# ramosian-glider/syzkaller

Hardware: AMD Instinct MI355X
Metric: coverage PCs triaged/sec vs corpus signal (+ % HBM roofline), 1/2/4/8 MI355X (higher is better)
Workload: dtype u32

## Files before the change

syzkaller_amd/csrc/sg_bucket.hip:

```cpp
#include "sg_part.h"

namespace sg {

#ifndef SG_BTHREADS
#define SG_BTHREADS 512
#endif
constexpr int kBThreads = SG_BTHREADS;
constexpr int kBWaves = kBThreads == 512 ? 6 : 8;
constexpr int kBU = 4;
constexpr uint32_t kHash = 8192;
constexpr uint32_t kMaxProbe = 31;
constexpr uint32_t kEmpty = 0xFFFFFFFFu;

struct BucketArgs {
  const uint32_t* in;
  const uint4* bdesc;
  const uint32_t* gbnd;
  uint32_t NG;
  uint32_t* mwords;
  const uint32_t* owords;
  uint32_t* nwords;
  uint8_t* rec_new;
  uint32_t* spill;
  uint32_t* nspill;
// ... 700 lines not shown
    cus = 256;
  const uint32_t grid = (uint32_t)(per_cu * cus);
  cache[key] = grid;
  return grid;
}

constexpr double kFsQueued = 0.9997;
static bool fs_split(sg_ctx* ctx) {
  const int64_t o = ctx->opt[kOptFlagSkip];
  if (o >= 0) return o != 0;
  m0f_poll(ctx);
  return ctx->m0f_queued >= kFsQueued;
}

int buckets_one(sg_ctx* ctx, const BucketPlan& bp, uint32_t* mwords, uint32_t* nwords, uint8_t* d_rec_new,
                const EmitArgs* emit, const uint32_t* owords) {
  const uint64_t nrec = bp.nrec;
  const uint32_t* gcount = bp.at<uint32_t>(ctx, kCB) + bp.ng;
  uint4* bdesc = bp.at<uint4>(ctx, kBD);
  uint32_t* nspill = bp.at<uint32_t>(ctx, kSP);
  const bool dbg = ctx->debug_part;
  BucketArgs ba{};
  ba.in = bp.at<uint32_t>(ctx, kV2);
  ba.bdesc = bdesc;
  ba.gbnd = bp.at<uint32_t>(ctx, kGB);
  ba.NG = (uint32_t)bp.NG;
  ba.mwords = mwords;
  ba.owords = owords;
  ba.nwords = nwords;
  ba.rec_new = d_rec_new;
  ba.nspill = nspill;
// ... 7 lines not shown
    ba.shard_cnt = emit->shard_cnt;
    ba.update = emit->update ? 1u : 0u;
    ba.gcur = emit->gcur;
    ba.goff = emit->goff;
  }
  uint32_t bgrid = persistent_grid(ctx, (const void*)k_bucket<false, 0>, kBThreads);
  const int64_t cap_blocks = ctx->opt[kOptBucketBlocks];
  if (cap_blocks > 0 && (uint64_t)cap_blocks < bgrid) bgrid = (uint32_t)cap_blocks;
  uint64_t* ddbg = nullptr;
  if (dbg) {
    SG_HIP(hipMalloc(&ddbg, (size_t)bgrid * 88));
    ba.dbg = ddbg;
  }
  const bool split = !emit && !dbg && d_rec_new && nrec <= kMaxLaunchRecords && fs_split(ctx);
  uint32_t* fsum = ba.ticket + 4;
  uint32_t* fcnt = (uint32_t*)ctx->dscal + 33;
  if (split) {
    if (!ctx->fs_ev) SG_HIP(hipEventCreateWithFlags(&ctx->fs_ev, hipEventDisableTiming));
    int rc = m0f_host_alloc(ctx);
    if (rc) return rc;
    SG_HIP(hipMemsetAsync(fcnt, 0, 4, ctx->stream));
  }
  SG_HIP(hipMemsetAsync(ba.ticket, 0, split ? 16 + kFsWords * 4 : 4, ctx->stream));
  SG_HIP(hipMemsetAsync(nspill, 0, 4, ctx->stream));
  ba.blist_b = bp.at<uint32_t>(ctx, kLB);
  ba.blist_q = bp.at<uint4>(ctx, kLQ);
  ba.nlist = bp.at<uint32_t>(ctx, kBP) + kNumBuckets;
  {
    ScopedTimer tm(ctx, "bucket_triage");
    if (split) {
      ba.win = 1;
      ba.win_shift = (uint32_t)ctx->opt[kOptFlagSkipSplit];
    }
    auto kb = emit  ? (emit->gcur ? k_bucket<false, 2> : k_bucket<false, 1>)
              : dbg ? k_bucket<true, 0>
                    : k_bucket<false, 0>;
    hipLaunchKernelGGL(kb, dim3(bgrid), dim3(kBThreads), 0, ctx->stream, ba);
    if (split) {
      hipLaunchKernelGGL(k_flag_summary, dim3(div_up(div_up(nrec, kFsRecs), 4)), dim3(256), 0, ctx->stream,
// ... 73 lines not shown
```

syzkaller_amd/csrc/sg_part.h:

```cpp
#pragma once

#include <algorithm>

#include "sg_internal.h"

namespace sg {

#ifndef SG_PT
#define SG_PT 16384
#endif
#ifndef SG_PTHREADS
#define SG_PTHREADS 1024
#endif
constexpr int kPT = SG_PT;
constexpr int kPThreads = SG_PTHREADS;
constexpr uint32_t kRecCap = 256;
constexpr uint32_t kGroupBits = 16;
constexpr uint32_t kGroupRecs = 1u << kGroupBits;
constexpr uint32_t kMaxGroups = 256;
static_assert(kGroupRecs % kRecCap == 0, "group boundaries must be tile cuts");
constexpr uint32_t kNumBuckets = 1u << 16;
constexpr uint32_t kBucketWords = 2048;
static_assert(kMaxLaunchRecords == (uint64_t)kMaxGroups * kGroupRecs, "records per partitioned launch");

// ... 19 lines not shown
}

constexpr uint32_t kFsBits = 12, kFsRecs = 1u << kFsBits;
constexpr uint32_t kFsWords = (uint32_t)(kMaxLaunchRecords >> kFsBits) / 32;
static_assert(kFsWords * 32ull * kFsRecs == kMaxLaunchRecords, "summary covers a launch's records");

constexpr uint64_t kSliceEntries = 1ull << 30;

struct RecSlice {
  uint64_t r0, r1, e0, e1;
};

enum Region : int {
  kTS, kTR, kGT,
  kH1, kO1, kV1, kB1,
  kNC, kCB,
  kCS, kCG, kCF,
  kCD, kDT,
  kBD, kGB,
  kH2, kO2, kV2,
  kSP, kTK,
  kBN, kBP,
  kLB, kLQ,
  kSC, kKM,
  kRegions
};
static_assert(kRegions <= sizeof(WsPlan::off) / sizeof(size_t), "the plan's regions fit WsPlan");

struct BucketPlan {
  uint64_t n, nrec, nA, nB, T, NG, ng, gmax;
  WsPlan p;
  size_t base = 0;
  BucketPlan(uint64_t n_, uint64_t nrec_);
  void rebase(size_t b) { base += b; }
  template <typename E>
  E* at(sg_ctx* ctx, Region r) const { return (E*)ws_at(ctx, base + p.off[r]); }
};

int partition_pass1(sg_ctx* ctx, const uint32_t* d_vals, const uint64_t* d_off, size_t ws_base, bool reserved,
                    BucketPlan& bp, bool trace, bool plane);
int partition_pass2(sg_ctx* ctx, const BucketPlan& bp, bool plane = true);
int partition_one(sg_ctx* ctx, const uint32_t* d_vals, const uint64_t* d_off, size_t ws_base, bool reserved,
                  BucketPlan& bp, bool trace = false);
int buckets_one(sg_ctx* ctx, const BucketPlan& bp, uint32_t* mwords, uint32_t* nwords, uint8_t* d_rec_new,
                const EmitArgs* emit, const uint32_t* owords = nullptr);
int m0_filter(sg_ctx* ctx, const BucketPlan& bp, uint32_t* mwords, uint32_t* nwords, uint8_t* d_rec_new, bool* done);
bool m0f_try(sg_ctx* ctx);
void m0f_poll(sg_ctx* ctx);
int m0f_note_partitioned(sg_ctx* ctx, const uint8_t* d_rec_new, uint64_t nrec);
int m0f_host_alloc(sg_ctx* ctx);
int record_slices(sg_ctx* ctx, const uint64_t* d_off, uint64_t nrec, std::vector<RecSlice>& out,
                  uint64_t lim = kSliceEntries);
int bucket_triage_one(sg_ctx* ctx, uint32_t* mwords, uint32_t* nwords, const uint32_t* d_vals, const uint64_t* d_off,
                      uint64_t n, uint64_t nrec, uint8_t* d_rec_new, const EmitArgs* emit = nullptr, size_t ws_base = 0,
                      bool trace = false);

}
```

syzkaller_amd/csrc/sg_part_triage.hip:

```cpp
#include "sg_part.h"

namespace sg {

int bucket_triage_one(sg_ctx* ctx, uint32_t* mwords, uint32_t* nwords, const uint32_t* d_vals, const uint64_t* d_off,
                      uint64_t n, uint64_t nrec, uint8_t* d_rec_new, const EmitArgs* emit, size_t ws_base, bool trace) {
  if (n == 0) return SG_OK;
  if (nrec == 0) {
    set_error("bucket triage: signal entries without records");
    return SG_EINVAL;
  }
  BucketPlan bp(n, nrec);
  if (emit || ws_base) {
    int rc = partition_one(ctx, d_vals, d_off, ws_base, ws_base != 0, bp, trace);
    if (rc) return rc;
    return buckets_one(ctx, bp, mwords, nwords, d_rec_new, emit);
  }
  const bool filter = m0f_try(ctx);
  int rc = partition_pass1(ctx, d_vals, d_off, 0, false, bp, trace, !filter);
  if (rc) return rc;
  if (filter) {
    bool done = false;
    rc = m0_filter(ctx, bp, mwords, nwords, d_rec_new, &done);
    if (rc || done) return rc;
  }
  rc = partition_pass2(ctx, bp, !filter);
  if (!rc) rc = buckets_one(ctx, bp, mwords, nwords, d_rec_new, nullptr);
  if (!rc) rc = m0f_note_partitioned(ctx, d_rec_new, nrec);
  return rc;
}

__global__ void k_rebase(const uint64_t* __restrict__ off, uint64_t n, uint64_t base, uint64_t* __restrict__ out) {
  const uint64_t i = (uint64_t)blockIdx.x * blockDim.x + threadIdx.x;
  if (i < n) out[i] = off[i] - base;
}

int rebase_offsets(sg_ctx* ctx, const uint64_t* d_off, uint64_t n, uint64_t base, uint64_t* d_out) {
  hipLaunchKernelGGL(k_rebase, dim3(div_up(n, 256)), dim3(256), 0, ctx->stream, d_off, n, base, d_out);
  SG_HIP(hipGetLastError());
  return SG_OK;
}

// ... 92 lines not shown

int record_slice_cuts(sg_ctx* ctx, const uint64_t* d_off, uint64_t nrec, uint64_t lim, std::vector<uint64_t>& cuts) {
  std::vector<RecSlice> sl;
  const int rc = record_slices(ctx, d_off, nrec, sl, lim);
  cuts.clear();
  for (const RecSlice& x : sl) cuts.insert(cuts.end(), {x.r0, x.r1, x.e0, x.e1});
  return rc;
}

int bucket_triage(sg_ctx* ctx, uint32_t* mwords, uint32_t* nwords, const uint32_t* d_vals, const uint64_t* d_off,
                  uint64_t n, uint64_t nrec, uint8_t* d_rec_new, bool trace) {
  if (nrec >= 0xFFFFFFFFull || n >= 0xFFFFFFFFull - 2 * kPT) {
    set_error("bucket triage: a batch holds < 2^32 signal entries and < 2^32 - 1 records");
    return SG_EINVAL;
  }
  if (nrec) SG_HIP(hipMemsetAsync(d_rec_new, 0, nrec, ctx->stream));
  const uint64_t m = ctx->max_launch_recs;
  if (nrec <= m && n <= kSliceEntries)
    return bucket_triage_one(ctx, mwords, nwords, d_vals, d_off, n, nrec, d_rec_new, nullptr, 0, trace);
  std::vector<RecSlice> sl;
  int rc = record_slices(ctx, d_off, nrec, sl);
  if (rc) return rc;
  const size_t need = nrec + sl.size();
  if (ctx->slice_off_cap < need) {
    SG_HIP(hipStreamSynchronize(ctx->stream));
    if (ctx->slice_off) SG_HIP(hipFree(ctx->slice_off));
    ctx->slice_off = nullptr;
    ctx->slice_off_cap = 0;
    SG_HIP(hipMalloc(&ctx->slice_off, need * 8));
    ctx->slice_off_cap = need;
  }
  size_t at = 0;
  for (const RecSlice& x : sl) {
    const uint64_t nr = x.r1 - x.r0;
// ... 38 lines not shown
```

syzkaller_amd/csrc/sg_partition.hip:

```cpp
#include "sg_part.h"

namespace sg {

constexpr int kPWaves = kPThreads / 64;
constexpr int kPerWave = kPT / kPWaves;
constexpr int kSteps = kPerWave / 64;

__device__ __forceinline__ uint32_t xcd_tile(uint32_t bid, uint32_t g) {
  const uint32_t x = bid & 7, q = g >> 3, r = g & 7;
  return (x < r ? x * (q + 1) : r * (q + 1) + (x - r) * q) + (bid >> 3);
}

struct Cuts {
  uint64_t nA, step, nB, n;
  const uint64_t* rec_off;
  uint64_t nrec;
  uint32_t* start;
  uint32_t* aux;
  __device__ __forceinline__ uint64_t B(uint64_t j) const { return rec_off[(j + 1) * kRecCap]; }
  __device__ __forceinline__ uint64_t countB(uint64_t x) const {
    uint64_t lo = 0, hi = nB;
    while (lo < hi) {
      const uint64_t mid = (lo + hi) >> 1;
      if (B(mid) < x)
        lo = mid + 1;
      else
        hi = mid;
    }
    return lo;
  }
};

__global__ void k_cuts(Cuts c) {
  const uint64_t i = (uint64_t)blockIdx.x * blockDim.x + threadIdx.x;
  const uint64_t total = c.nA + c.nB;
  if (i > total) return;
  if (i == total) {
    c.start[total] = (uint32_t)c.n;
    return;
  }
  uint64_t x, rank;
  if (i < c.nA) {
    x = i * c.step;
    rank = i + c.countB(x);
  } else {
    const uint64_t j = i - c.nA;
    x = c.B(j);
    const uint64_t a = x / c.step + 1;
    rank = j + (a < c.nA ? a : c.nA);
  }
  c.start[rank] = (uint32_t)x;
  const uint64_t xe = x < c.n ? x : (c.n ? c.n - 1 : 0);
  c.aux[rank] = (uint32_t)sgd::seg_search(c.rec_off, 0, c.nrec - 1, xe);
}

__global__ void k_group_tiles(const uint64_t* __restrict__ rec_off, uint64_t nA, uint32_t NG, uint32_t T,
                              uint32_t* __restrict__ gt) {
  const uint32_t g = blockIdx.x * blockDim.x + threadIdx.x;
  if (g > NG) return;
  if (g == 0 || g == NG) {
    gt[g] = g ? T : 0u;
    return;
  }
  const uint64_t a = rec_off[(uint64_t)g * kGroupRecs] / kPT + 1;
  gt[g] = (uint32_t)((uint64_t)g * (kGroupRecs / kRecCap) - 1 + (a < nA ? a : nA));
}

__device__ __forceinline__ uint32_t group_start(const uint32_t* goff1, uint32_t T, uint32_t NG, const uint32_t* gt,
                                                uint64_t j) {
  return goff1[(j / NG) * T + gt[j % NG]];
}

__global__ void k_group_chunks(const uint32_t* __restrict__ goff1, uint32_t T, uint32_t NG,
                               const uint32_t* __restrict__ gt, uint64_t ng, uint32_t* __restrict__ nch) {
  const uint64_t j = (uint64_t)blockIdx.x * blockDim.x + threadIdx.x;
  if (j >= ng) return;
  const uint32_t sz = group_start(goff1, T, NG, gt, j + 1) - group_start(goff1, T, NG, gt, j);
  nch[j] = (sz + kPT - 1) / kPT;
}

__global__ void k_chunk_list(const uint32_t* __restrict__ goff1, uint32_t T, uint32_t NG,
                             const uint32_t* __restrict__ gt, uint64_t ng,
                             const uint32_t* __restrict__ cbase, uint64_t gmax, uint32_t* __restrict__ cstart,
                             uint32_t* __restrict__ cgov, uint32_t* __restrict__ cfirst) {
  const uint64_t i = (uint64_t)blockIdx.x * blockDim.x + threadIdx.x;
  const uint32_t G = cbase[ng], n = goff1[256ull * T];
  if (i < ng) {
    const uint32_t g0 = group_start(goff1, T, NG, gt, i), g1 = group_start(goff1, T, NG, gt, i + 1);
    uint32_t c = cbase[i];
    for (uint32_t e = g0; e < g1; e += kPT, c++) {
      cstart[c] = e;
      cgov[c] = (uint32_t)i;
    }
  }
  if (i >= G && i <= gmax) {
    cstart[i] = n;
    cgov[i] = (uint32_t)(ng - 1);
  }
  if (i <= 256) cfirst[i] = i < 256 ? cbase[i * NG] : G;
}


__global__ void k_chunk_desc(const uint32_t* __restrict__ cstart, const uint32_t* __restrict__ cgov,
                             const uint32_t* __restrict__ gcount, uint64_t gmax, const uint32_t* __restrict__ goff1,
                             uint32_t T, uint32_t NG, const uint32_t* __restrict__ gt, uint4* __restrict__ desc,
                             uint2* __restrict__ dtile) {
  const uint64_t bid = (uint64_t)blockIdx.x * blockDim.x + threadIdx.x;
  if (bid >= gmax) return;
  const uint32_t G = *gcount;
  if (bid < G) {
    const uint32_t c = xcd_tile((uint32_t)bid, G), s0 = cstart[c], s1 = cstart[c + 1], j = cgov[c];
    const uint32_t* row = goff1 + (uint64_t)(j / NG) * T;
    const uint32_t lo = gt[j % NG], hi = gt[j % NG + 1];
    desc[bid] = make_uint4(s0, s1, j, c);
    dtile[bid] = make_uint2(last_le(row, lo, hi, s0), last_le(row, lo, hi, s1 - 1) + 1);
  } else {
    desc[bid] = make_uint4(0, 0, 0, 0);
    dtile[bid] = make_uint2(0, 0);
  }
}

constexpr int kHistQ = kPT / 4 / kPThreads;

__global__ __launch_bounds__(kPThreads) void k_p1_hist(const uint32_t* __restrict__ v,
                                                       const uint32_t* __restrict__ start, uint32_t* __restrict__ hist) {
  __shared__ uint32_t cnt[256];
// ... 519 lines not shown
__global__ __launch_bounds__(kPThreads) __attribute__((amdgpu_waves_per_eu(8, 8))) void k_p2_scatter(P2Args a) {
  __shared__ uint32_t stage[kPT];
  __shared__ uint32_t cnt[256];
  __shared__ uint32_t gbase[256];
  __shared__ SegLds<uint16_t> L;
  const uint4 dsc = a.desc[blockIdx.x];
  const uint2 dt = a.dtile[blockIdx.x];
  const uint32_t s0 = dsc.x, s1 = dsc.y;
  if (s0 >= s1) return;
  if (s1 - s0 == (uint32_t)kPT)
    p2_chunk<true>(a, stage, cnt, gbase, L, s0, s1, dsc.z, dsc.w, dt);
  else
    p2_chunk<false>(a, stage, cnt, gbase, L, s0, s1, dsc.z, dsc.w, dt);
}

__global__ void k_bucket_compact(const uint4* __restrict__ bdesc, const uint32_t* __restrict__ lpos,
                                 uint32_t* __restrict__ blist_b, uint4* __restrict__ blist_q) {
  const uint32_t b = blockIdx.x * blockDim.x + threadIdx.x;
  if (b >= kNumBuckets) return;
  const uint4 q = bdesc[b];
  if (q.x < q.y) {
    blist_b[lpos[b]] = b;
    blist_q[lpos[b]] = q;
  }
}

__global__ void k_bucket_desc(const uint32_t* __restrict__ goff2, const uint32_t* __restrict__ gcount,
                              const uint32_t* __restrict__ cfirst, uint4* __restrict__ bdesc, uint32_t* __restrict__ nz) {
  const uint32_t b = blockIdx.x * blockDim.x + threadIdx.x;
  if (b >= kNumBuckets) return;
  const uint32_t d = b >> 8, f = b & 255, c0 = cfirst[d], nch = cfirst[d + 1] - c0;
  const uint32_t* row = goff2 + (uint64_t)f * *gcount + c0;
  const uint32_t lo = row[0], hi = row[nch];
  bdesc[b] = make_uint4(lo, hi, c0, nch);
  nz[b] = lo < hi ? 1u : 0u;
}

__global__ void k_bucket_groups(const uint32_t* __restrict__ goff2, const uint32_t* __restrict__ gcount,
                                const uint32_t* __restrict__ cbase, uint32_t NG, uint32_t* __restrict__ gbnd) {
  const uint64_t i = (uint64_t)blockIdx.x * blockDim.x + threadIdx.x;
  if (i >= (uint64_t)kNumBuckets * NG) return;
  const uint32_t b = (uint32_t)(i / NG), g = (uint32_t)(i % NG);
  gbnd[i] = goff2[(uint64_t)(b & 255) * *gcount + cbase[(b >> 8) * NG + g]];
}

__global__ void k_top_plane(const uint32_t* __restrict__ v1, uint64_t n, uint8_t* __restrict__ b1) {
  for (uint64_t i = ((uint64_t)blockIdx.x * blockDim.x + threadIdx.x) * 4; i < n;
       i += (uint64_t)gridDim.x * blockDim.x * 4) {
    if (i + 4 <= n && ((uintptr_t)(v1 + i) & 15) == 0) {
      const uint4 q = *reinterpret_cast<const uint4*>(v1 + i);
      *reinterpret_cast<uint32_t*>(b1 + i) = (q.x >> 24) | ((q.y >> 24) << 8) | ((q.z >> 24) << 16) | (q.w & 0xFF000000u);
    } else {
      for (uint64_t k = i; k < i + 4 && k < n; k++) b1[k] = (uint8_t)(v1[k] >> 24);
    }
  }
}

constexpr int kScanThreads = 1024;
constexpr int kScanPer = 16;
constexpr uint32_t kScanTile = kScanThreads * kScanPer;

__device__ __forceinline__ uint32_t block_excl_scan(uint32_t v, uint32_t* wsum, uint32_t* total) {
  const int tid = threadIdx.x, lane = tid & 63, w = tid >> 6;
  uint32_t incl = v;
#pragma unroll
  for (int o = 1; o < 64; o <<= 1) {
    const uint32_t y = __shfl_up(incl, o);
    if (lane >= o) incl += y;
  }
  if (lane == 63) wsum[w] = incl;
  __syncthreads();
  if (tid < 64) {
    const uint32_t x = tid < (int)(blockDim.x >> 6) ? wsum[tid] : 0u;
    uint32_t wi = x;
#pragma unroll
    for (int o = 1; o < 64; o <<= 1) {
      const uint32_t y = __shfl_up(wi, o);
      if (lane >= o) wi += y;
    }
    if (tid < (int)(blockDim.x >> 6)) wsum[tid] = wi - x;
    if (tid == 63) *total = wi;
  }
  __syncthreads();
  return wsum[w] + incl - v;
}
// ... 14 lines not shown
    for (int k = 0; k < kScanPer; k++) {
      const uint64_t i = base + (uint64_t)k * kScanThreads + threadIdx.x;
      s += i < n ? in[i] : 0u;
    }
  }
  for (int o = 32; o; o >>= 1) s += __shfl_down(s, o);
  if ((threadIdx.x & 63) == 0) wsum[threadIdx.x >> 6] = s;
  __syncthreads();
  if (threadIdx.x == 0) {
    uint32_t t = 0;
    for (int w = 0; w < kScanThreads / 64; w++) t += wsum[w];
    sums[blockIdx.x] = t;
  }
}

__global__ __launch_bounds__(kScanThreads) void k_scan32_top(uint32_t* __restrict__ sums, uint64_t nb) {
  __shared__ uint32_t wsum[16];
  __shared__ uint32_t tot;
  uint32_t carry = 0;
  for (uint64_t b0 = 0; b0 < nb; b0 += kScanThreads) {
    const uint64_t i = b0 + threadIdx.x;
    const uint32_t v = i < nb ? sums[i] : 0u;
    const uint32_t ex = block_excl_scan(v, wsum, &tot);
    if (i < nb) sums[i] = carry + ex;
    carry += tot;
    __syncthreads();
  }
}

__global__ __launch_bounds__(kScanThreads) void k_scan32_apply(const uint32_t* __restrict__ in, uint64_t n,
                                                               const uint32_t* __restrict__ n_dev, uint32_t mul,
                                                               const uint32_t* __restrict__ sums,
                                                               uint32_t* __restrict__ out) {
  __shared__ uint32_t wsum[16];
  __shared__ uint32_t tot;
  n = scan_n(n, n_dev, mul);
  const uint64_t b_last = n ? (n - 1) / kScanTile : 0;
  if (blockIdx.x > b_last) return;
  const uint64_t base = (uint64_t)blockIdx.x * kScanTile + (uint64_t)threadIdx.x * kScanPer;
  const bool full = base + kScanPer <= n;
  uint32_t v[kScanPer];
  uint32_t s = 0;
  if (full) {
#pragma unroll
    for (int k = 0; k < kScanPer; k += 4) {
      const uint4 q = *reinterpret_cast<const uint4*>(in + base + k);
      v[k] = q.x;
      v[k + 1] = q.y;
      v[k + 2] = q.z;
      v[k + 3] = q.w;
    }
  } else {
#pragma unroll
    for (int k = 0; k < kScanPer; k++) v[k] = base + k < n ? in[base + k] : 0u;
  }
#pragma unroll
  for (int k = 0; k < kScanPer; k++) s += v[k];
  uint32_t run = (sums ? sums[blockIdx.x] : 0u) + block_excl_scan(s, wsum, &tot);
  uint32_t o[kScanPer];
#pragma unroll
  for (int k = 0; k < kScanPer; k++) {
    o[k] = run;
    run += v[k];
  }
  if (full) {
#pragma unroll
    for (int k = 0; k < kScanPer; k += 4)
      *reinterpret_cast<uint4*>(out + base + k) = make_uint4(o[k], o[k + 1], o[k + 2], o[k + 3]);
  } else {
#pragma unroll
    for (int k = 0; k < kScanPer; k++)
      if (base + k < n) out[base + k] = o[k];
  }
// ... 6 lines not shown
                  const uint32_t* n_dev = nullptr, uint32_t mul = 1) {
  ScopedTimer tm(ctx, "scan");
  const uint64_t nb = (n + kScanTile - 1) / kScanTile;
  if (nb == 0) {
    SG_HIP(hipMemsetAsync(out, 0, 4, ctx->stream));
    return SG_OK;
  }
  if (nb == 1) {
    hipLaunchKernelGGL(k_scan32_apply, dim3(1), dim3(kScanThreads), 0, ctx->stream, in, n, n_dev, mul,
                       (const uint32_t*)nullptr, out);
    SG_HIP(hipGetLastError());
    return SG_OK;
  }
  hipLaunchKernelGGL(k_scan32_reduce, dim3((uint32_t)nb), dim3(kScanThreads), 0, ctx->stream, in, n, n_dev, mul,
                     scratch);
  hipLaunchKernelGGL(k_scan32_top, dim3(1), dim3(kScanThreads), 0, ctx->stream, scratch, nb);
  hipLaunchKernelGGL(k_scan32_apply, dim3((uint32_t)nb), dim3(kScanThreads), 0, ctx->stream, in, n, n_dev, mul,
                     scratch, out);
  SG_HIP(hipGetLastError());
  return SG_OK;
}

BucketPlan::BucketPlan(uint64_t n_, uint64_t nrec_) : n(n_), nrec(nrec_) {
  nA = (n + kPT - 1) / kPT;
  nB = nrec ? (nrec - 1) / kRecCap : 0;
  T = nA + nB;
  NG = nrec ? (nrec - 1) / kGroupRecs + 1 : 1;
  ng = 256 * NG;
  gmax = ng + nA;
  const uint64_t nb = kNumBuckets;
  const size_t bytes[] = {
      (T + 1) * 4, (T + 1) * 4, (NG + 1) * 4,
      256 * T * 4, (256 * T + 1) * 4, n * 4, n + 64,
      ng * 4, (ng + 1) * 4,
      (gmax + 1) * 4, (gmax + 1) * 4, 257 * 4,
      gmax * 16, gmax * 8,
      nb * 16, nb * NG * 4,
      256 * gmax * 4, (256 * gmax + 1) * 4, n * 4 + 64,
      (nb + 1) * 4, 16 + kFsWords * 4,
      nb * 4, (nb + 1) * 4,
      nb * 4, nb * 16,
      scan32_ws(256 * (gmax > T ? gmax : T)), T * (kPT / 8),
  };
  static_assert(sizeof(bytes) / sizeof(bytes[0]) == kRegions, "one size per region");
  for (size_t b : bytes) p.add(b);
}

size_t bucket_plan_bytes(uint64_t n, uint64_t nrec) { return BucketPlan(n, nrec).p.total; }

int partition_pass1(sg_ctx* ctx, const uint32_t* d_vals, const uint64_t* d_off, size_t ws_base, bool reserved,
                    BucketPlan& bp, bool trace, bool plane) {
  if (256 * bp.gmax >= 0xFFFFFFFFull || bp.NG > kMaxGroups) {
    set_error("bucket triage: batch too large");
    return SG_EINVAL;
  }
  int rc = reserved ? SG_OK : ws_reserve(ctx, ws_base + bp.p.total);
  if (rc) return rc;
  if (ctx->ws_cap < ws_base + bp.p.total) {
    set_error("bucket triage: workspace not reserved");
    return SG_EINVAL;
  }
  bp.rebase(ws_base);
  uint32_t* tstart = bp.at<uint32_t>(ctx, kTS);
  uint32_t* trec = bp.at<uint32_t>(ctx, kTR);
  uint32_t* hist1 = bp.at<uint32_t>(ctx, kH1);
  uint32_t* goff1 = bp.at<uint32_t>(ctx, kO1);
  uint64_t* keep = bp.at<uint64_t>(ctx, kKM);
  const uint32_t T = (uint32_t)bp.T, NG = (uint32_t)bp.NG;
  const bool dbg = ctx->debug_part;
  const Cuts c1{bp.nA, kPT, bp.nB, bp.n, d_off, bp.nrec, tstart, trec};
  hipLaunchKernelGGL(k_cuts, dim3(div_up(bp.T + 1, 256)), dim3(256), 0, ctx->stream, c1);
  hipLaunchKernelGGL(k_group_tiles, dim3(div_up(bp.NG + 1, 256)), dim3(256), 0, ctx->stream, d_off, bp.nA, NG, T,
                     bp.at<uint32_t>(ctx, kGT));
  {
    ScopedTimer tm(ctx, "p1_hist");
    if (trace)
      hipLaunchKernelGGL(k_hist_trace, dim3(T), dim3(kPThreads), 0, ctx->stream, d_vals, d_off, bp.nrec,
                         (const uint32_t*)tstart, (const uint32_t*)trec, T, hist1, keep);
    else if (((uintptr_t)d_vals & 15) == 0)
      hipLaunchKernelGGL(k_hist_rep<false>, dim3(T), dim3(kPThreads), 0, ctx->stream, d_vals,
                         (const uint32_t*)tstart, (const uint4*)nullptr, T, (const uint32_t*)nullptr, hist1);
    else
      hipLaunchKernelGGL(k_p1_hist, dim3(T), dim3(kPThreads), 0, ctx->stream, d_vals,
                         (const uint32_t*)tstart, hist1);
  }
  rc = scan32(ctx, hist1, goff1, 256 * bp.T, bp.at<uint32_t>(ctx, kSC));
  if (rc) return rc;
  P1Args a1{d_vals, d_off, bp.nrec, tstart, trec, T, goff1, hist1, bp.at<uint32_t>(ctx, kV1),
// ... 9 lines not shown
    auto k1 = dbg ? (trace ? k_p1_scatter<true, true> : k_p1_scatter<true, false>)
                  : (trace ? k_p1_scatter<false, true> : k_p1_scatter<false, false>);
    hipLaunchKernelGGL(k1, dim3(T), dim3(kPThreads), 0, ctx->stream, a1);
  }
  if (dbg) {
    unsigned long long h[8];
    SG_HIP(hipMemcpy(h, p1dbg, 64, hipMemcpyDeviceToHost));
    SG_HIP(hipFree(p1dbg));
    fprintf(stderr, "sg p1_scatter per tile (cycles, wave 0): load+meta %.0f build+lookup %.0f rank %.0f stage %.0f "
            "write %.0f (tiles %llu)\n", (double)h[0] / h[5], (double)h[1] / h[5], (double)h[2] / h[5],
            (double)h[3] / h[5], (double)h[4] / h[5], h[5]);
  }
  return SG_OK;
}

int partition_pass2(sg_ctx* ctx, const BucketPlan& bp, bool plane) {
  const uint32_t* gt = bp.at<uint32_t>(ctx, kGT);
  const uint32_t* goff1 = bp.at<uint32_t>(ctx, kO1);
  uint32_t* v1 = bp.at<uint32_t>(ctx, kV1);
  uint8_t* b1 = bp.at<uint8_t>(ctx, kB1);
  uint32_t* nch = bp.at<uint32_t>(ctx, kNC);
  uint32_t* cbase = bp.at<uint32_t>(ctx, kCB);
  uint32_t* cstart = bp.at<uint32_t>(ctx, kCS);
  uint32_t* cgov = bp.at<uint32_t>(ctx, kCG);
  uint32_t* cfirst = bp.at<uint32_t>(ctx, kCF);
  uint4* cdesc = bp.at<uint4>(ctx, kCD);
  uint2* dtile = bp.at<uint2>(ctx, kDT);
  uint4* bdesc = bp.at<uint4>(ctx, kBD);
  uint32_t* hist2 = bp.at<uint32_t>(ctx, kH2);
  uint32_t* goff2 = bp.at<uint32_t>(ctx, kO2);
  uint32_t* scr = bp.at<uint32_t>(ctx, kSC);
  uint32_t* bnz = bp.at<uint32_t>(ctx, kBN);
  uint32_t* blpos = bp.at<uint32_t>(ctx, kBP);
  const uint32_t T = (uint32_t)bp.T, G = (uint32_t)bp.gmax, NG = (uint32_t)bp.NG;
  const uint32_t* gcount = cbase + bp.ng;
  if (!plane) {
    hipLaunchKernelGGL(k_top_plane, dim3((uint32_t)std::min<uint64_t>(4096, div_up(bp.n, 1024))), dim3(256), 0,
                       ctx->stream, (const uint32_t*)v1, bp.n, b1);
    SG_HIP(hipGetLastError());
  }
  hipLaunchKernelGGL(k_group_chunks, dim3(div_up(bp.ng, 256)), dim3(256), 0, ctx->stream, goff1, T, NG, gt, bp.ng,
                     nch);
  int rc = scan32(ctx, nch, cbase, bp.ng, scr);
  if (rc) return rc;
  hipLaunchKernelGGL(k_chunk_list, dim3(div_up((bp.ng > bp.gmax ? bp.ng : bp.gmax) + 1, 256)), dim3(256), 0,
                     ctx->stream, goff1, T, NG, gt, bp.ng, (const uint32_t*)cbase, bp.gmax, cstart, cgov, cfirst);
  hipLaunchKernelGGL(k_chunk_desc, dim3(div_up(bp.gmax, 256)), dim3(256), 0, ctx->stream, (const uint32_t*)cstart,
                     (const uint32_t*)cgov, gcount, bp.gmax, goff1, T, NG, gt, cdesc, dtile);
  {
    ScopedTimer tm(ctx, "p2_hist");
    hipLaunchKernelGGL(k_hist_bytes, dim3(G), dim3(kHBThreads), 0, ctx->stream, (const uint8_t*)b1,
                       (const uint4*)cdesc, gcount, hist2);
  }
  rc = scan32(ctx, hist2, goff2, 256 * bp.gmax, scr, gcount, 256);
  if (rc) return rc;
  P2Args a2{v1, cdesc, dtile, gcount, goff1, bp.at<uint32_t>(ctx, kTR), T, NG, goff2, hist2, bp.at<uint32_t>(ctx, kV2)};
  {
    ScopedTimer tm(ctx, "p2_scatter");
    hipLaunchKernelGGL(k_p2_scatter, dim3(G), dim3(kPThreads), 0, ctx->stream, a2);
  }
  hipLaunchKernelGGL(k_bucket_desc, dim3(kNumBuckets / 256), dim3(256), 0, ctx->stream, (const uint32_t*)goff2,
                     gcount, (const uint32_t*)cfirst, bdesc, bnz);
  hipLaunchKernelGGL(k_bucket_groups, dim3(div_up((uint64_t)kNumBuckets * NG, 256)), dim3(256), 0, ctx->stream,
                     (const uint32_t*)goff2, gcount, (const uint32_t*)cbase, NG, bp.at<uint32_t>(ctx, kGB));
  rc = scan32(ctx, bnz, blpos, kNumBuckets, scr);
  if (rc) return rc;
  hipLaunchKernelGGL(k_bucket_compact, dim3(kNumBuckets / 256), dim3(256), 0, ctx->stream, (const uint4*)bdesc,
                     (const uint32_t*)blpos, bp.at<uint32_t>(ctx, kLB), bp.at<uint4>(ctx, kLQ));
  SG_HIP(hipGetLastError());
  return SG_OK;
}

int partition_one(sg_ctx* ctx, const uint32_t* d_vals, const uint64_t* d_off, size_t ws_base, bool reserved,
                  BucketPlan& bp, bool trace) {
  const int rc = partition_pass1(ctx, d_vals, d_off, ws_base, reserved, bp, trace, true);
  return rc ? rc : partition_pass2(ctx, bp);
}

}
```

Baseline: 134.7 billion.

## Fuse partition bookkeeping kernels and fold memsets into kernels to cut launches

Merges the cut and group-tile kernels into one launch, which also zeroes the record-new flags in place of a separate memset. The chunk count, scan and list kernels become a single-block chunk kernel, with chunk descriptors found by binary search over the chunk bases. The bucket descriptor, group, scan and compact steps become two kernels that use per-block counts, and the ticket, spill and flag-count scalars are zeroed inside them, so the memsets in buckets_one are skipped. The top-level scan kernel is removed by having each apply block sum the preceding block totals itself. The goal is fewer small launches and memsets per batch, at the cost of a serial single-block chunk scan and redundant prefix summation in each block.

```diff
diff --git a/syzkaller_amd/csrc/sg_bucket.hip b/syzkaller_amd/csrc/sg_bucket.hip
--- a/syzkaller_amd/csrc/sg_bucket.hip
+++ b/syzkaller_amd/csrc/sg_bucket.hip
@@ -738,7 +738,7 @@
 }
 
 int buckets_one(sg_ctx* ctx, const BucketPlan& bp, uint32_t* mwords, uint32_t* nwords, uint8_t* d_rec_new,
-                const EmitArgs* emit, const uint32_t* owords) {
+                const EmitArgs* emit, const uint32_t* owords, bool scalars_zeroed) {
   const uint64_t nrec = bp.nrec;
   const uint32_t* gcount = bp.at<uint32_t>(ctx, kCB) + bp.ng;
   uint4* bdesc = bp.at<uint4>(ctx, kBD);
@@ -776,15 +776,17 @@
   }
   const bool split = !emit && !dbg && d_rec_new && nrec <= kMaxLaunchRecords && fs_split(ctx);
   uint32_t* fsum = ba.ticket + 4;
-  uint32_t* fcnt = (uint32_t*)ctx->dscal + 33;
+  uint32_t* fcnt = fs_count(ctx);
   if (split) {
     if (!ctx->fs_ev) SG_HIP(hipEventCreateWithFlags(&ctx->fs_ev, hipEventDisableTiming));
     int rc = m0f_host_alloc(ctx);
     if (rc) return rc;
-    SG_HIP(hipMemsetAsync(fcnt, 0, 4, ctx->stream));
-  }
-  SG_HIP(hipMemsetAsync(ba.ticket, 0, split ? 16 + kFsWords * 4 : 4, ctx->stream));
-  SG_HIP(hipMemsetAsync(nspill, 0, 4, ctx->stream));
+    if (!scalars_zeroed) SG_HIP(hipMemsetAsync(fcnt, 0, 4, ctx->stream));
+  }
+  if (!scalars_zeroed) {
+    SG_HIP(hipMemsetAsync(ba.ticket, 0, split ? 16 + kFsWords * 4 : 4, ctx->stream));
+    SG_HIP(hipMemsetAsync(nspill, 0, 4, ctx->stream));
+  }
   ba.blist_b = bp.at<uint32_t>(ctx, kLB);
   ba.blist_q = bp.at<uint4>(ctx, kLQ);
   ba.nlist = bp.at<uint32_t>(ctx, kBP) + kNumBuckets;
diff --git a/syzkaller_amd/csrc/sg_part.h b/syzkaller_amd/csrc/sg_part.h
--- a/syzkaller_amd/csrc/sg_part.h
+++ b/syzkaller_amd/csrc/sg_part.h
@@ -57,8 +57,8 @@
 enum Region : int {
   kTS, kTR, kGT,
   kH1, kO1, kV1, kB1,
-  kNC, kCB,
-  kCS, kCG, kCF,
+  kCB,
+  kCF,
   kCD, kDT,
   kBD, kGB,
   kH2, kO2, kV2,
@@ -81,12 +81,13 @@
 };
 
 int partition_pass1(sg_ctx* ctx, const uint32_t* d_vals, const uint64_t* d_off, size_t ws_base, bool reserved,
-                    BucketPlan& bp, bool trace, bool plane);
-int partition_pass2(sg_ctx* ctx, const BucketPlan& bp, bool plane = true);
+                    BucketPlan& bp, bool trace, bool plane, uint8_t* clear_flags = nullptr);
+int partition_pass2(sg_ctx* ctx, const BucketPlan& bp, bool plane = true, uint32_t* zero_fcnt = nullptr);
 int partition_one(sg_ctx* ctx, const uint32_t* d_vals, const uint64_t* d_off, size_t ws_base, bool reserved,
                   BucketPlan& bp, bool trace = false);
 int buckets_one(sg_ctx* ctx, const BucketPlan& bp, uint32_t* mwords, uint32_t* nwords, uint8_t* d_rec_new,
-                const EmitArgs* emit, const uint32_t* owords = nullptr);
+                const EmitArgs* emit, const uint32_t* owords = nullptr, bool scalars_zeroed = false);
+inline uint32_t* fs_count(sg_ctx* ctx) { return (uint32_t*)ctx->dscal + 33; }
 int m0_filter(sg_ctx* ctx, const BucketPlan& bp, uint32_t* mwords, uint32_t* nwords, uint8_t* d_rec_new, bool* done);
 bool m0f_try(sg_ctx* ctx);
 void m0f_poll(sg_ctx* ctx);
@@ -96,6 +97,6 @@
                   uint64_t lim = kSliceEntries);
 int bucket_triage_one(sg_ctx* ctx, uint32_t* mwords, uint32_t* nwords, const uint32_t* d_vals, const uint64_t* d_off,
                       uint64_t n, uint64_t nrec, uint8_t* d_rec_new, const EmitArgs* emit = nullptr, size_t ws_base = 0,
-                      bool trace = false);
+                      bool trace = false, bool clear_flags = false);
 
 }
diff --git a/syzkaller_amd/csrc/sg_part_triage.hip b/syzkaller_amd/csrc/sg_part_triage.hip
--- a/syzkaller_amd/csrc/sg_part_triage.hip
+++ b/syzkaller_amd/csrc/sg_part_triage.hip
@@ -3,7 +3,8 @@
 namespace sg {
 
 int bucket_triage_one(sg_ctx* ctx, uint32_t* mwords, uint32_t* nwords, const uint32_t* d_vals, const uint64_t* d_off,
-                      uint64_t n, uint64_t nrec, uint8_t* d_rec_new, const EmitArgs* emit, size_t ws_base, bool trace) {
+                      uint64_t n, uint64_t nrec, uint8_t* d_rec_new, const EmitArgs* emit, size_t ws_base, bool trace,
+                      bool clear_flags) {
   if (n == 0) return SG_OK;
   if (nrec == 0) {
     set_error("bucket triage: signal entries without records");
@@ -16,15 +17,15 @@
     return buckets_one(ctx, bp, mwords, nwords, d_rec_new, emit);
   }
   const bool filter = m0f_try(ctx);
-  int rc = partition_pass1(ctx, d_vals, d_off, 0, false, bp, trace, !filter);
+  int rc = partition_pass1(ctx, d_vals, d_off, 0, false, bp, trace, !filter, clear_flags ? d_rec_new : nullptr);
   if (rc) return rc;
   if (filter) {
     bool done = false;
     rc = m0_filter(ctx, bp, mwords, nwords, d_rec_new, &done);
     if (rc || done) return rc;
   }
-  rc = partition_pass2(ctx, bp, !filter);
-  if (!rc) rc = buckets_one(ctx, bp, mwords, nwords, d_rec_new, nullptr);
+  rc = partition_pass2(ctx, bp, !filter, fs_count(ctx));
+  if (!rc) rc = buckets_one(ctx, bp, mwords, nwords, d_rec_new, nullptr, nullptr, true);
   if (!rc) rc = m0f_note_partitioned(ctx, d_rec_new, nrec);
   return rc;
 }
@@ -147,10 +148,10 @@
     set_error("bucket triage: a batch holds < 2^32 signal entries and < 2^32 - 1 records");
     return SG_EINVAL;
   }
-  if (nrec) SG_HIP(hipMemsetAsync(d_rec_new, 0, nrec, ctx->stream));
   const uint64_t m = ctx->max_launch_recs;
-  if (nrec <= m && n <= kSliceEntries)
-    return bucket_triage_one(ctx, mwords, nwords, d_vals, d_off, n, nrec, d_rec_new, nullptr, 0, trace);
+  const bool one = nrec <= m && n <= kSliceEntries;
+  if (nrec && !(one && n)) SG_HIP(hipMemsetAsync(d_rec_new, 0, nrec, ctx->stream));
+  if (one) return bucket_triage_one(ctx, mwords, nwords, d_vals, d_off, n, nrec, d_rec_new, nullptr, 0, trace, true);
   std::vector<RecSlice> sl;
   int rc = record_slices(ctx, d_off, nrec, sl);
   if (rc) return rc;
diff --git a/syzkaller_amd/csrc/sg_partition.hip b/syzkaller_amd/csrc/sg_partition.hip
--- a/syzkaller_amd/csrc/sg_partition.hip
+++ b/syzkaller_amd/csrc/sg_partition.hip
@@ -31,8 +31,7 @@
   }
 };
 
-__global__ void k_cuts(Cuts c) {
-  const uint64_t i = (uint64_t)blockIdx.x * blockDim.x + threadIdx.x;
+__device__ __forceinline__ void cut_one(const Cuts& c, uint64_t i) {
   const uint64_t total = c.nA + c.nB;
   if (i > total) return;
   if (i == total) {
@@ -54,16 +53,30 @@
   c.aux[rank] = (uint32_t)sgd::seg_search(c.rec_off, 0, c.nrec - 1, xe);
 }
 
-__global__ void k_group_tiles(const uint64_t* __restrict__ rec_off, uint64_t nA, uint32_t NG, uint32_t T,
-                              uint32_t* __restrict__ gt) {
-  const uint32_t g = blockIdx.x * blockDim.x + threadIdx.x;
+__device__ __forceinline__ void group_tile(const Cuts& c, uint32_t NG, uint32_t g, uint32_t* __restrict__ gt) {
   if (g > NG) return;
   if (g == 0 || g == NG) {
-    gt[g] = g ? T : 0u;
+    gt[g] = g ? (uint32_t)(c.nA + c.nB) : 0u;
     return;
   }
-  const uint64_t a = rec_off[(uint64_t)g * kGroupRecs] / kPT + 1;
-  gt[g] = (uint32_t)((uint64_t)g * (kGroupRecs / kRecCap) - 1 + (a < nA ? a : nA));
+  const uint64_t a = c.rec_off[(uint64_t)g * kGroupRecs] / kPT + 1;
+  gt[g] = (uint32_t)((uint64_t)g * (kGroupRecs / kRecCap) - 1 + (a < c.nA ? a : c.nA));
+}
+
+__global__ void k_tiles(Cuts c, uint32_t NG, uint32_t* __restrict__ gt, uint8_t* __restrict__ rec_new,
+                        uint64_t nclear) {
+  const uint64_t i = (uint64_t)blockIdx.x * blockDim.x + threadIdx.x, nthr = (uint64_t)gridDim.x * blockDim.x;
+  cut_one(c, i);
+  group_tile(c, NG, (uint32_t)(i < NG + 1 ? i : NG + 1), gt);
+  if (rec_new) {
+    uint64_t head = (16 - ((uintptr_t)rec_new & 15)) & 15;
+    head = head < nclear ? head : nclear;
+    const uint64_t nq = (nclear - head) / 16, tail = head + nq * 16;
+    uint4* q = reinterpret_cast<uint4*>(rec_new + head);
+    for (uint64_t k = i; k < nq; k += nthr) q[k] = make_uint4(0, 0, 0, 0);
+    if (i < head) rec_new[i] = 0;
+    if (i < nclear - tail) rec_new[tail + i] = 0;
+  }
 }
 
 __device__ __forceinline__ uint32_t group_start(const uint32_t* goff1, uint32_t T, uint32_t NG, const uint32_t* gt,
@@ -71,45 +84,56 @@
   return goff1[(j / NG) * T + gt[j % NG]];
 }
 
-__global__ void k_group_chunks(const uint32_t* __restrict__ goff1, uint32_t T, uint32_t NG,
-                               const uint32_t* __restrict__ gt, uint64_t ng, uint32_t* __restrict__ nch) {
-  const uint64_t j = (uint64_t)blockIdx.x * blockDim.x + threadIdx.x;
-  if (j >= ng) return;
-  const uint32_t sz = group_start(goff1, T, NG, gt, j + 1) - group_start(goff1, T, NG, gt, j);
-  nch[j] = (sz + kPT - 1) / kPT;
-}
-
-__global__ void k_chunk_list(const uint32_t* __restrict__ goff1, uint32_t T, uint32_t NG,
-                             const uint32_t* __restrict__ gt, uint64_t ng,
-                             const uint32_t* __restrict__ cbase, uint64_t gmax, uint32_t* __restrict__ cstart,
-                             uint32_t* __restrict__ cgov, uint32_t* __restrict__ cfirst) {
-  const uint64_t i = (uint64_t)blockIdx.x * blockDim.x + threadIdx.x;
-  const uint32_t G = cbase[ng], n = goff1[256ull * T];
-  if (i < ng) {
-    const uint32_t g0 = group_start(goff1, T, NG, gt, i), g1 = group_start(goff1, T, NG, gt, i + 1);
-    uint32_t c = cbase[i];
-    for (uint32_t e = g0; e < g1; e += kPT, c++) {
-      cstart[c] = e;
-      cgov[c] = (uint32_t)i;
-    }
-  }
-  if (i >= G && i <= gmax) {
-    cstart[i] = n;
-    cgov[i] = (uint32_t)(ng - 1);
-  }
-  if (i <= 256) cfirst[i] = i < 256 ? cbase[i * NG] : G;
-}
-
-
-__global__ void k_chunk_desc(const uint32_t* __restrict__ cstart, const uint32_t* __restrict__ cgov,
-                             const uint32_t* __restrict__ gcount, uint64_t gmax, const uint32_t* __restrict__ goff1,
-                             uint32_t T, uint32_t NG, const uint32_t* __restrict__ gt, uint4* __restrict__ desc,
-                             uint2* __restrict__ dtile) {
+__device__ __forceinline__ uint32_t block_excl_scan(uint32_t v, uint32_t* wsum, uint32_t* total, uint32_t p = 0,
+                                                    uint32_t* psum = nullptr);
+
+constexpr int kChunkJ = 4;
+__global__ __launch_bounds__(1024) void k_chunks(const uint32_t* __restrict__ goff1, uint32_t T, uint32_t NG,
+                                                 const uint32_t* __restrict__ gt, uint64_t ng,
+                                                 uint32_t* __restrict__ cbase, uint32_t* __restrict__ cfirst) {
+  __shared__ uint32_t wsum[16];
+  __shared__ uint32_t tot;
+  uint32_t carry = 0;
+  for (uint64_t j0 = 0; j0 < ng; j0 += (uint64_t)blockDim.x * kChunkJ) {
+    const uint64_t jb = j0 + (uint64_t)threadIdx.x * kChunkJ;
+    uint32_t gs[kChunkJ + 1];
+#pragma unroll
+    for (int k = 0; k <= kChunkJ; k++) gs[k] = group_start(goff1, T, NG, gt, jb + k < ng ? jb + k : ng);
+    uint32_t nc[kChunkJ], s = 0;
+#pragma unroll
+    for (int k = 0; k < kChunkJ; k++) {
+      nc[k] = (gs[k + 1] - gs[k] + kPT - 1) / kPT;
+      s += nc[k];
+    }
+    uint32_t c = carry + block_excl_scan(s, wsum, &tot);
+#pragma unroll
+    for (int k = 0; k < kChunkJ; k++) {
+      const uint64_t j = jb + k;
+      if (j < ng) {
+        cbase[j] = c;
+        if (j % NG == 0) cfirst[j / NG] = c;
+      }
+      c += nc[k];
+    }
+    carry += tot;
+    __syncthreads();
+  }
+  if (threadIdx.x == 0) {
+    cbase[ng] = carry;
+    cfirst[256] = carry;
+  }
+}
+
+__global__ void k_chunk_desc(const uint32_t* __restrict__ cbase, uint64_t ng, uint64_t gmax,
+                             const uint32_t* __restrict__ goff1, uint32_t T, uint32_t NG,
+                             const uint32_t* __restrict__ gt, uint4* __restrict__ desc, uint2* __restrict__ dtile) {
   const uint64_t bid = (uint64_t)blockIdx.x * blockDim.x + threadIdx.x;
   if (bid >= gmax) return;
-  const uint32_t G = *gcount;
+  const uint32_t G = cbase[ng];
   if (bid < G) {
-    const uint32_t c = xcd_tile((uint32_t)bid, G), s0 = cstart[c], s1 = cstart[c + 1], j = cgov[c];
+    const uint32_t c = xcd_tile((uint32_t)bid, G), j = last_le(cbase, 0, (uint32_t)ng, c);
+    const uint32_t s0 = group_start(goff1, T, NG, gt, j) + (c - cbase[j]) * (uint32_t)kPT;
+    const uint32_t e = group_start(goff1, T, NG, gt, (uint64_t)j + 1), s1 = e - s0 < (uint32_t)kPT ? e : s0 + kPT;
     const uint32_t* row = goff1 + (uint64_t)(j / NG) * T;
     const uint32_t lo = gt[j % NG], hi = gt[j % NG + 1];
     desc[bid] = make_uint4(s0, s1, j, c);
@@ -659,34 +683,66 @@
     p2_chunk<false>(a, stage, cnt, gbase, L, s0, s1, dsc.z, dsc.w, dt);
 }
 
-__global__ void k_bucket_compact(const uint4* __restrict__ bdesc, const uint32_t* __restrict__ lpos,
-                                 uint32_t* __restrict__ blist_b, uint4* __restrict__ blist_q) {
-  const uint32_t b = blockIdx.x * blockDim.x + threadIdx.x;
-  if (b >= kNumBuckets) return;
-  const uint4 q = bdesc[b];
-  if (q.x < q.y) {
-    blist_b[lpos[b]] = b;
-    blist_q[lpos[b]] = q;
-  }
-}
-
-__global__ void k_bucket_desc(const uint32_t* __restrict__ goff2, const uint32_t* __restrict__ gcount,
-                              const uint32_t* __restrict__ cfirst, uint4* __restrict__ bdesc, uint32_t* __restrict__ nz) {
-  const uint32_t b = blockIdx.x * blockDim.x + threadIdx.x;
-  if (b >= kNumBuckets) return;
-  const uint32_t d = b >> 8, f = b & 255, c0 = cfirst[d], nch = cfirst[d + 1] - c0;
-  const uint32_t* row = goff2 + (uint64_t)f * *gcount + c0;
+constexpr int kTabThreads = 1024;
+constexpr uint32_t kTabBlocks = kNumBuckets / kTabThreads;
+static_assert(kTabBlocks <= 64, "k_bucket_list folds the block counts in one wave");
+
+__global__ __launch_bounds__(kTabThreads) void k_bucket_tables(const uint32_t* __restrict__ goff2,
+                                                               const uint32_t* __restrict__ gcount,
+                                                               const uint32_t* __restrict__ cfirst,
+                                                               const uint32_t* __restrict__ cbase, uint32_t NG,
+                                                               uint4* __restrict__ bdesc, uint32_t* __restrict__ gbnd,
+                                                               uint32_t* __restrict__ nzsum) {
+  __shared__ uint32_t wcnt[kTabThreads / 64];
+  const uint32_t G = *gcount;
+  const uint64_t i = (uint64_t)blockIdx.x * kTabThreads + threadIdx.x;
+  if (i < (uint64_t)kNumBuckets * NG) {
+    const uint32_t b = (uint32_t)(i / NG), g = (uint32_t)(i % NG);
+    gbnd[i] = goff2[(uint64_t)(b & 255) * G + cbase[(b >> 8) * NG + g]];
+  }
+  if (blockIdx.x >= kTabBlocks) return;
+  const uint32_t b = (uint32_t)i, d = b >> 8, f = b & 255, c0 = cfirst[d], nch = cfirst[d + 1] - c0;
+  const uint32_t* row = goff2 + (uint64_t)f * G + c0;
   const uint32_t lo = row[0], hi = row[nch];
   bdesc[b] = make_uint4(lo, hi, c0, nch);
-  nz[b] = lo < hi ? 1u : 0u;
-}
-
-__global__ void k_bucket_groups(const uint32_t* __restrict__ goff2, const uint32_t* __restrict__ gcount,
-                                const uint32_t* __restrict__ cbase, uint32_t NG, uint32_t* __restrict__ gbnd) {
-  const uint64_t i = (uint64_t)blockIdx.x * blockDim.x + threadIdx.x;
-  if (i >= (uint64_t)kNumBuckets * NG) return;
-  const uint32_t b = (uint32_t)(i / NG), g = (uint32_t)(i % NG);
-  gbnd[i] = goff2[(uint64_t)(b & 255) * *gcount + cbase[(b >> 8) * NG + g]];
+  const uint32_t c = (uint32_t)__popcll(__ballot(lo < hi));
+  if ((threadIdx.x & 63) == 0) wcnt[threadIdx.x >> 6] = c;
+  __syncthreads();
+  if (threadIdx.x == 0) {
+    uint32_t t = 0;
+    for (int w = 0; w < kTabThreads / 64; w++) t += wcnt[w];
+    nzsum[blockIdx.x] = t;
+  }
+}
+
+__global__ __launch_bounds__(kTabThreads) void k_bucket_list(const uint4* __restrict__ bdesc,
+                                                             const uint32_t* __restrict__ nzsum,
+                                                             uint32_t* __restrict__ blist_b,
+                                                             uint4* __restrict__ blist_q, uint32_t* __restrict__ nlist,
+                                                             uint32_t* __restrict__ ticket,
+                                                             uint32_t* __restrict__ nspill,
+                                                             uint32_t* __restrict__ fcnt) {
+  __shared__ uint32_t wsum[kTabThreads / 64];
+  __shared__ uint32_t psum[kTabThreads / 64];
+  __shared__ uint32_t tot;
+  const uint32_t b = blockIdx.x * kTabThreads + threadIdx.x;
+  const uint4 q = bdesc[b];
+  const uint32_t nz = q.x < q.y ? 1u : 0u;
+  const uint32_t p = threadIdx.x < blockIdx.x ? nzsum[threadIdx.x] : 0u;
+  uint32_t pos = block_excl_scan(nz, wsum, &tot, p, psum);
+  for (int w = 0; w < kTabThreads / 64; w++) pos += psum[w];
+  if (nz) {
+    blist_b[pos] = b;
+    blist_q[pos] = q;
+  }
+  if (b == kNumBuckets - 1) *nlist = pos + nz;
+  if (ticket && blockIdx.x == 0) {
+    for (uint32_t k = threadIdx.x; k < 4 + kFsWords; k += kTabThreads) ticket[k] = 0;
+    if (threadIdx.x == 0) {
+      *nspill = 0;
+      *fcnt = 0;
+    }
+  }
 }
 
 __global__ void k_top_plane(const uint32_t* __restrict__ v1, uint64_t n, uint8_t* __restrict__ b1) {
@@ -705,7 +761,8 @@
 constexpr int kScanPer = 16;
 constexpr uint32_t kScanTile = kScanThreads * kScanPer;
 
-__device__ __forceinline__ uint32_t block_excl_scan(uint32_t v, uint32_t* wsum, uint32_t* total) {
+__device__ __forceinline__ uint32_t block_excl_scan(uint32_t v, uint32_t* wsum, uint32_t* total, uint32_t p,
+                                                    uint32_t* psum) {
   const int tid = threadIdx.x, lane = tid & 63, w = tid >> 6;
   uint32_t incl = v;
 #pragma unroll
@@ -714,6 +771,10 @@
     if (lane >= o) incl += y;
   }
   if (lane == 63) wsum[w] = incl;
+  if (psum) {
+    for (int o = 32; o; o >>= 1) p += __shfl_down(p, o);
+    if (lane == 0) psum[w] = p;
+  }
   __syncthreads();
   if (tid < 64) {
     const uint32_t x = tid < (int)(blockDim.x >> 6) ? wsum[tid] : 0u;
@@ -758,29 +819,19 @@
   }
 }
 
-__global__ __launch_bounds__(kScanThreads) void k_scan32_top(uint32_t* __restrict__ sums, uint64_t nb) {
-  __shared__ uint32_t wsum[16];
-  __shared__ uint32_t tot;
-  uint32_t carry = 0;
-  for (uint64_t b0 = 0; b0 < nb; b0 += kScanThreads) {
-    const uint64_t i = b0 + threadIdx.x;
-    const uint32_t v = i < nb ? sums[i] : 0u;
-    const uint32_t ex = block_excl_scan(v, wsum, &tot);
-    if (i < nb) sums[i] = carry + ex;
-    carry += tot;
-    __syncthreads();
-  }
-}
-
 __global__ __launch_bounds__(kScanThreads) void k_scan32_apply(const uint32_t* __restrict__ in, uint64_t n,
                                                                const uint32_t* __restrict__ n_dev, uint32_t mul,
                                                                const uint32_t* __restrict__ sums,
                                                                uint32_t* __restrict__ out) {
   __shared__ uint32_t wsum[16];
+  __shared__ uint32_t psum[16];
   __shared__ uint32_t tot;
   n = scan_n(n, n_dev, mul);
   const uint64_t b_last = n ? (n - 1) / kScanTile : 0;
   if (blockIdx.x > b_last) return;
+  uint32_t p = 0;
+  if (sums)
+    for (uint32_t i = threadIdx.x; i < blockIdx.x; i += kScanThreads) p += sums[i];
   const uint64_t base = (uint64_t)blockIdx.x * kScanTile + (uint64_t)threadIdx.x * kScanPer;
   const bool full = base + kScanPer <= n;
   uint32_t v[kScanPer];
@@ -800,7 +851,9 @@
   }
 #pragma unroll
   for (int k = 0; k < kScanPer; k++) s += v[k];
-  uint32_t run = (sums ? sums[blockIdx.x] : 0u) + block_excl_scan(s, wsum, &tot);
+  uint32_t run = block_excl_scan(s, wsum, &tot, p, psum);
+#pragma unroll
+  for (int w = 0; w < kScanThreads / 64; w++) run += psum[w];
   uint32_t o[kScanPer];
 #pragma unroll
   for (int k = 0; k < kScanPer; k++) {
@@ -837,7 +890,6 @@
   }
   hipLaunchKernelGGL(k_scan32_reduce, dim3((uint32_t)nb), dim3(kScanThreads), 0, ctx->stream, in, n, n_dev, mul,
                      scratch);
-  hipLaunchKernelGGL(k_scan32_top, dim3(1), dim3(kScanThreads), 0, ctx->stream, scratch, nb);
   hipLaunchKernelGGL(k_scan32_apply, dim3((uint32_t)nb), dim3(kScanThreads), 0, ctx->stream, in, n, n_dev, mul,
                      scratch, out);
   SG_HIP(hipGetLastError());
@@ -855,8 +907,8 @@
   const size_t bytes[] = {
       (T + 1) * 4, (T + 1) * 4, (NG + 1) * 4,
       256 * T * 4, (256 * T + 1) * 4, n * 4, n + 64,
-      ng * 4, (ng + 1) * 4,
-      (gmax + 1) * 4, (gmax + 1) * 4, 257 * 4,
+      (ng + 1) * 4,
+      257 * 4,
       gmax * 16, gmax * 8,
       nb * 16, nb * NG * 4,
       256 * gmax * 4, (256 * gmax + 1) * 4, n * 4 + 64,
@@ -872,7 +924,7 @@
 size_t bucket_plan_bytes(uint64_t n, uint64_t nrec) { return BucketPlan(n, nrec).p.total; }
 
 int partition_pass1(sg_ctx* ctx, const uint32_t* d_vals, const uint64_t* d_off, size_t ws_base, bool reserved,
-                    BucketPlan& bp, bool trace, bool plane) {
+                    BucketPlan& bp, bool trace, bool plane, uint8_t* clear_flags) {
   if (256 * bp.gmax >= 0xFFFFFFFFull || bp.NG > kMaxGroups) {
     set_error("bucket triage: batch too large");
     return SG_EINVAL;
@@ -892,9 +944,8 @@
   const uint32_t T = (uint32_t)bp.T, NG = (uint32_t)bp.NG;
   const bool dbg = ctx->debug_part;
   const Cuts c1{bp.nA, kPT, bp.nB, bp.n, d_off, bp.nrec, tstart, trec};
-  hipLaunchKernelGGL(k_cuts, dim3(div_up(bp.T + 1, 256)), dim3(256), 0, ctx->stream, c1);
-  hipLaunchKernelGGL(k_group_tiles, dim3(div_up(bp.NG + 1, 256)), dim3(256), 0, ctx->stream, d_off, bp.nA, NG, T,
-                     bp.at<uint32_t>(ctx, kGT));
+  hipLaunchKernelGGL(k_tiles, dim3(div_up(std::max(bp.T, bp.NG) + 1, 256)), dim3(256), 0, ctx->stream, c1, NG,
+                     bp.at<uint32_t>(ctx, kGT), clear_flags, bp.nrec);
   {
     ScopedTimer tm(ctx, "p1_hist");
     if (trace)
@@ -934,15 +985,12 @@
   return SG_OK;
 }
 
-int partition_pass2(sg_ctx* ctx, const BucketPlan& bp, bool plane) {
+int partition_pass2(sg_ctx* ctx, const BucketPlan& bp, bool plane, uint32_t* zero_fcnt) {
   const uint32_t* gt = bp.at<uint32_t>(ctx, kGT);
   const uint32_t* goff1 = bp.at<uint32_t>(ctx, kO1);
   uint32_t* v1 = bp.at<uint32_t>(ctx, kV1);
   uint8_t* b1 = bp.at<uint8_t>(ctx, kB1);
-  uint32_t* nch = bp.at<uint32_t>(ctx, kNC);
   uint32_t* cbase = bp.at<uint32_t>(ctx, kCB);
-  uint32_t* cstart = bp.at<uint32_t>(ctx, kCS);
-  uint32_t* cgov = bp.at<uint32_t>(ctx, kCG);
   uint32_t* cfirst = bp.at<uint32_t>(ctx, kCF);
   uint4* cdesc = bp.at<uint4>(ctx, kCD);
   uint2* dtile = bp.at<uint2>(ctx, kDT);
@@ -950,7 +998,6 @@
   uint32_t* hist2 = bp.at<uint32_t>(ctx, kH2);
   uint32_t* goff2 = bp.at<uint32_t>(ctx, kO2);
   uint32_t* scr = bp.at<uint32_t>(ctx, kSC);
-  uint32_t* bnz = bp.at<uint32_t>(ctx, kBN);
   uint32_t* blpos = bp.at<uint32_t>(ctx, kBP);
   const uint32_t T = (uint32_t)bp.T, G = (uint32_t)bp.gmax, NG = (uint32_t)bp.NG;
   const uint32_t* gcount = cbase + bp.ng;
@@ -959,34 +1006,28 @@
                        ctx->stream, (const uint32_t*)v1, bp.n, b1);
     SG_HIP(hipGetLastError());
   }
-  hipLaunchKernelGGL(k_group_chunks, dim3(div_up(bp.ng, 256)), dim3(256), 0, ctx->stream, goff1, T, NG, gt, bp.ng,
-                     nch);
-  int rc = scan32(ctx, nch, cbase, bp.ng, scr);
-  if (rc) return rc;
-  hipLaunchKernelGGL(k_chunk_list, dim3(div_up((bp.ng > bp.gmax ? bp.ng : bp.gmax) + 1, 256)), dim3(256), 0,
-                     ctx->stream, goff1, T, NG, gt, bp.ng, (const uint32_t*)cbase, bp.gmax, cstart, cgov, cfirst);
-  hipLaunchKernelGGL(k_chunk_desc, dim3(div_up(bp.gmax, 256)), dim3(256), 0, ctx->stream, (const uint32_t*)cstart,
-                     (const uint32_t*)cgov, gcount, bp.gmax, goff1, T, NG, gt, cdesc, dtile);
+  hipLaunchKernelGGL(k_chunks, dim3(1), dim3(1024), 0, ctx->stream, goff1, T, NG, gt, bp.ng, cbase, cfirst);
+  hipLaunchKernelGGL(k_chunk_desc, dim3(div_up(bp.gmax, 256)), dim3(256), 0, ctx->stream, (const uint32_t*)cbase,
+                     bp.ng, bp.gmax, goff1, T, NG, gt, cdesc, dtile);
   {
     ScopedTimer tm(ctx, "p2_hist");
     hipLaunchKernelGGL(k_hist_bytes, dim3(G), dim3(kHBThreads), 0, ctx->stream, (const uint8_t*)b1,
                        (const uint4*)cdesc, gcount, hist2);
   }
-  rc = scan32(ctx, hist2, goff2, 256 * bp.gmax, scr, gcount, 256);
+  int rc = scan32(ctx, hist2, goff2, 256 * bp.gmax, scr, gcount, 256);
   if (rc) return rc;
   P2Args a2{v1, cdesc, dtile, gcount, goff1, bp.at<uint32_t>(ctx, kTR), T, NG, goff2, hist2, bp.at<uint32_t>(ctx, kV2)};
   {
     ScopedTimer tm(ctx, "p2_scatter");
     hipLaunchKernelGGL(k_p2_scatter, dim3(G), dim3(kPThreads), 0, ctx->stream, a2);
   }
-  hipLaunchKernelGGL(k_bucket_desc, dim3(kNumBuckets / 256), dim3(256), 0, ctx->stream, (const uint32_t*)goff2,
-                     gcount, (const uint32_t*)cfirst, bdesc, bnz);
-  hipLaunchKernelGGL(k_bucket_groups, dim3(div_up((uint64_t)kNumBuckets * NG, 256)), dim3(256), 0, ctx->stream,
-                     (const uint32_t*)goff2, gcount, (const uint32_t*)cbase, NG, bp.at<uint32_t>(ctx, kGB));
-  rc = scan32(ctx, bnz, blpos, kNumBuckets, scr);
-  if (rc) return rc;
-  hipLaunchKernelGGL(k_bucket_compact, dim3(kNumBuckets / 256), dim3(256), 0, ctx->stream, (const uint4*)bdesc,
-                     (const uint32_t*)blpos, bp.at<uint32_t>(ctx, kLB), bp.at<uint4>(ctx, kLQ));
+  hipLaunchKernelGGL(k_bucket_tables, dim3(kTabBlocks * NG), dim3(kTabThreads), 0, ctx->stream,
+                     (const uint32_t*)goff2, gcount, (const uint32_t*)cfirst, (const uint32_t*)cbase, NG, bdesc,
+                     bp.at<uint32_t>(ctx, kGB), blpos);
+  uint32_t* nspill = bp.at<uint32_t>(ctx, kSP);
+  hipLaunchKernelGGL(k_bucket_list, dim3(kTabBlocks), dim3(kTabThreads), 0, ctx->stream, (const uint4*)bdesc,
+                     (const uint32_t*)blpos, bp.at<uint32_t>(ctx, kLB), bp.at<uint4>(ctx, kLQ), blpos + kNumBuckets,
+                     zero_fcnt ? bp.at<uint32_t>(ctx, kTK) : nullptr, nspill, zero_fcnt);
   SG_HIP(hipGetLastError());
   return SG_OK;
 }
```

After: 133.7 billion. About the same (-0.7%).
